# mims-harvard/ProCyon

Measured on AMD Instinct MI355X. Metric: phenotype-gen tokens/sec (ProCyon-Full greedy generation, end to end), higher is better.
Workload: dtype bf16; 1 GPU; configs[1]: ProCyon-Full (ESM2-650M + Llama-3-8B geometry=full) bf16 batch=1, 1024-residue protein, 512-token prompt, 256-token greedy generation; parallelism=single GPU

## Files before the change

procyon_amd/csrc/pcy_elem.hip:

```cpp
#include "pcy_internal.h"
#include "pcy_pick.h"

namespace {

constexpr int NT = 256;

__global__ __launch_bounds__(NT) void rmsnorm_kernel(const bf16_t* __restrict__ x, const bf16_t* __restrict__ w,
                                                     bf16_t* __restrict__ y, int d, float eps, int cast) {
  __shared__ float red[NT / 64];
  const bf16_t* xr = x + (size_t)blockIdx.x * d;
  bf16_t* yr = y + (size_t)blockIdx.x * d;
  float ss = 0.f;
  for (int k = threadIdx.x * 8; k < d; k += NT * 8) {
    const uint4 v = *reinterpret_cast<const uint4*>(xr + k);
    const uint32_t u[4] = {v.x, v.y, v.z, v.w};
#pragma unroll
    for (int j = 0; j < 4; ++j) { float a = lo_bf(u[j]), b = hi_bf(u[j]); ss += a * a + b * b; }
  }
  ss = block_sum<NT>(ss, red);
  const float rstd = rsqrtf(ss / (float)d + eps);
  for (int k = threadIdx.x * 8; k < d; k += NT * 8) {
    const uint4 v = *reinterpret_cast<const uint4*>(xr + k);
    const uint4 g = *reinterpret_cast<const uint4*>(w + k);
    const uint32_t u[4] = {v.x, v.y, v.z, v.w}, gg[4] = {g.x, g.y, g.z, g.w};
// ... 323 lines not shown
  }
  __syncthreads();
  if (tp == 0 && live) {
#pragma unroll
    for (int e = 0; e < 8; ++e) {
      float a = acc[e];
      int n = cnt[e];
#pragma unroll
      for (int q = 0; q < 3; ++q) {
        if (mode == 2) a = fmaxf(a, part[q][fg][e]);
        else { a += part[q][fg][e]; n += pcnt[q][fg][e]; }
      }
      wsum[((size_t)p * POOL_CH + ch) * d + c + e] = a;
      wcnt[((size_t)p * POOL_CH + ch) * d + c + e] = n;
    }
  }
}
__global__ __launch_bounds__(NT) void pool_finish_kernel(const float* __restrict__ wsum, const int* __restrict__ wcnt, int d, int mode,
                                                         bf16_t* __restrict__ out) {
  const int p = blockIdx.x, c = blockIdx.y * NT + threadIdx.x;
  if (c >= d) return;
  float a = wsum[(size_t)p * POOL_CH * d + c];
  int n = wcnt[(size_t)p * POOL_CH * d + c];
  for (int ch = 1; ch < POOL_CH; ++ch) {
    const float v = wsum[((size_t)p * POOL_CH + ch) * d + c];
    if (mode == 2) a = fmaxf(a, v);
    else { a += v; n += wcnt[((size_t)p * POOL_CH + ch) * d + c]; }
  }
  out[(size_t)p * d + c] = (mode == 2) ? f2bf(a) : f2bf(rbf(a) / (float)n);
}


__global__ __launch_bounds__(PICK_NT) void pick_stage1_kernel(const bf16_t* __restrict__ logits, int V, PickPartial* __restrict__ part) {
  __shared__ float redv[PICK_NT / 64];
  __shared__ int redi[PICK_NT / 64];
  __shared__ float red[PICK_NT / 64];
  const int b = blockIdx.y, c = blockIdx.x;
  const int chunk = (V + PICK_NB - 1) / PICK_NB;
  const int lo = c * chunk, hi = (lo + chunk) < V ? (lo + chunk) : V;
  const bf16_t* lg = logits + (size_t)b * V;
  float best = -INFINITY;
  int bi = 0x7fffffff;
  for (int i = lo + threadIdx.x; i < hi; i += PICK_NT) {
    const float v = bf2f(lg[i]);
    if (v > best || (v == best && i < bi)) { best = v; bi = i; }
  }
#pragma unroll
  for (int o = 32; o > 0; o >>= 1) {
    const float ov = __shfl_xor(best, o, 64);
    const int oi = __shfl_xor(bi, o, 64);
    if (ov > best || (ov == best && oi < bi)) { best = ov; bi = oi; }
  }
  const int w = threadIdx.x >> 6;
  if ((threadIdx.x & 63) == 0) { redv[w] = best; redi[w] = bi; }
  __syncthreads();
  best = redv[0]; bi = redi[0];
  for (int i = 1; i < PICK_NT / 64; ++i)
    if (redv[i] > best || (redv[i] == best && redi[i] < bi)) { best = redv[i]; bi = redi[i]; }
  float se = 0.f;
  for (int i = lo + threadIdx.x; i < hi; i += PICK_NT) se += expf(bf2f(lg[i]) - best);
  se = block_sum<PICK_NT>(se, red);
  if (threadIdx.x == 0) part[b * PICK_NB + c] = PickPartial{best, bi, best > -INFINITY ? se : 0.f, 0};
}

__global__ __launch_bounds__(256) void pick_stage2_kernel(const bf16_t* __restrict__ logits, int V, const PickPartial* __restrict__ part,
                                                          int32_t* __restrict__ next_tok, int32_t* __restrict__ tokens_out, int max_steps,
                                                          float* __restrict__ logprob, int32_t* __restrict__ step_dev, int32_t* __restrict__ pos_dev,
                                                          int advance_pos, int B, PcyStop stop) {
  __shared__ int s_unfinished;
  const int l = threadIdx.x & 63;
  if (stop.finished) {
    if (*stop.done) return;
    if (threadIdx.x == 0) s_unfinished = 0;
    __syncthreads();
  }
  const int step = *step_dev;
  for (int b = threadIdx.x >> 6; b < B; b += 4) {
    if (stop.finished && stop.finished[b]) {
      if (l == 0) { next_tok[b] = stop.eos_id; tokens_out[(size_t)b * max_steps + step] = stop.eos_id; }
      continue;
    }
    float best, se;
    int bi;
    pick_merge_row(part[b * PICK_NB + l], best, bi, se);
    if (l == 0) {
      const float lsm = pick_logprob(logits + (size_t)b * V, bi, best, se);
      logprob[b] += lsm;
      next_tok[b] = bi;
      tokens_out[(size_t)b * max_steps + step] = bi;
      if (stop.finished) {
        if (bi == stop.eos_id) stop.finished[b] = 1;
        else atomicAdd(&s_unfinished, 1);
      }
    }
  }
  __syncthreads();
  if (threadIdx.x == 0) {
    if (advance_pos) *pos_dev += 1;
    *step_dev = step + 1;
    if (stop.finished && s_unfinished == 0) {
      if (stop.n_steps_run) *stop.n_steps_run = step + 1;
      *stop.done = 1;
    }
  }
}

constexpr int SMP_NT = 1024;

__global__ __launch_bounds__(PICK_NT) void sample_stage1_kernel(const bf16_t* __restrict__ logits, int V, float temperature,
                                                                float4* __restrict__ part) {
  __shared__ float red[PICK_NT / 64];
  const int b = blockIdx.y, c = blockIdx.x;
  const int chunk = (V + PICK_NB - 1) / PICK_NB;
  const int lo = c * chunk, hi = (lo + chunk) < V ? (lo + chunk) : V;
  const bf16_t* lg = logits + (size_t)b * V;
  const bool scaled = temperature != 1.0f;
  float mr = -INFINITY, ms = -INFINITY;
  for (int i = lo + threadIdx.x; i < hi; i += PICK_NT) {
    const float v = bf2f(lg[i]);
    mr = fmaxf(mr, v);
    ms = fmaxf(ms, scaled ? rbf(v / temperature) : v);
  }
  mr = block_max<PICK_NT>(mr, red);
  ms = block_max<PICK_NT>(ms, red);
  float sr = 0.f, ss = 0.f;
  for (int i = lo + threadIdx.x; i < hi; i += PICK_NT) {
    const float v = bf2f(lg[i]);
    sr += expf(v - mr);
    ss += expf((scaled ? rbf(v / temperature) : v) - ms);
  }
  sr = block_sum<PICK_NT>(sr, red);
  ss = block_sum<PICK_NT>(ss, red);
  if (threadIdx.x == 0) part[b * PICK_NB + c] = make_float4(mr, mr > -INFINITY ? sr : 0.f, ms, ms > -INFINITY ? ss : 0.f);
}

// ... 858 lines not shown
    int acc = 0;
    for (int q = 0; q < nseq; ++q) { out[q] = acc; acc += (cu[q + 1] - cu[q] + pad - 1) / pad * pad; }
    out[nseq] = acc;
  }
}
void pcy_launch_vt_offsets(hipStream_t s, const int32_t* cu, int nseq, int pad, int32_t* vt_cu_out) {
  hipLaunchKernelGGL(vt_offsets_kernel, dim3(1), dim3(64), 0, s, cu, nseq, pad, vt_cu_out);
}
void pcy_launch_transpose_v(hipStream_t s, const bf16_t* buf, int ld, int vcol0, int nh, int dh, const int32_t* cu,
                            const int32_t* vt_cu, int nseq, int max_len, bf16_t* vt, int vt_total) {
  if (nseq <= 0) return;
  const int maxpad = (max_len + 63) / 64 * 64;
  hipLaunchKernelGGL(transpose_v_kernel, dim3((maxpad + 63) / 64, nh * dh / 64, nseq), dim3(NT), 0, s, buf, ld, vcol0, dh, cu, vt_cu, vt, vt_total);
}
size_t pcy_pool_ws_bytes(int nprot, int d) { return (size_t)nprot * POOL_CH * d * 8; }
void pcy_launch_pool(hipStream_t s, const bf16_t* h, int d, const int32_t* seg, const int32_t* rng, int nprot, int mode, bf16_t* out,
                     void* ws) {
  if (nprot <= 0) return;
  float* wsum = reinterpret_cast<float*>(ws);
  int* wcnt = reinterpret_cast<int*>(wsum + (size_t)nprot * POOL_CH * d);
  hipLaunchKernelGGL(pool_partial_kernel, dim3(nprot, (d + 511) / 512, POOL_CH), dim3(NT), 0, s, h, d, seg, rng, mode, wsum, wcnt);
  hipLaunchKernelGGL(pool_finish_kernel, dim3(nprot, (d + NT - 1) / NT), dim3(NT), 0, s, wsum, wcnt, d, mode, out);
}
void pcy_launch_pick_stage1(hipStream_t s, const bf16_t* logits, int rows, int V, void* partials) {
  if (rows > 0) hipLaunchKernelGGL(pick_stage1_kernel, dim3(PICK_NB, rows), dim3(PICK_NT), 0, s, logits, V, reinterpret_cast<PickPartial*>(partials));
}
void pcy_launch_greedy_pick(hipStream_t s, const bf16_t* logits, int B, int V, int32_t* next_tok, int32_t* tokens_out,
                            int max_steps, float* logprob, int32_t* pos_dev, int32_t* step_dev, int advance_pos, void* partials,
                            const PcyStop& stop) {
  hipLaunchKernelGGL(pick_stage1_kernel, dim3(PICK_NB, B), dim3(PICK_NT), 0, s, logits, V, reinterpret_cast<PickPartial*>(partials));
  hipLaunchKernelGGL(pick_stage2_kernel, dim3(1), dim3(256), 0, s, logits, V, reinterpret_cast<const PickPartial*>(partials), next_tok,
                     tokens_out, max_steps, logprob, step_dev, pos_dev, advance_pos, B, stop);
}
int pcy_sample_max_vocab() { return SMP_NT * SMP_KMAX; }
void pcy_launch_sample_step(hipStream_t s, const bf16_t* logits, int B, int V, float temperature, float nucleus_p, const float* uniforms,
                            unsigned* hist, bf16_t* probs_out, int32_t* next_tok, int32_t* tokens_out, int max_steps, float* logprob,
                            int32_t* pos_dev, int32_t* step_dev, int advance_pos, void* partials, bf16_t* pbits, const PcyStop& stop) {
  hipLaunchKernelGGL(sample_stage1_kernel, dim3(PICK_NB, B), dim3(PICK_NT), 0, s, logits, V, temperature, reinterpret_cast<float4*>(partials));
  hipLaunchKernelGGL(sample_probs_kernel, dim3(PICK_NB, B), dim3(PICK_NT), 0, s, logits, V, reinterpret_cast<const float4*>(partials), temperature,
                     nucleus_p > 0.f ? 1 : 0, hist, pbits, stop, probs_out ? 1 : 0);
  hipLaunchKernelGGL(sample_stage2_kernel, dim3(B), dim3(SMP_NT), 0, s, logits, V, reinterpret_cast<const float4*>(partials), temperature,
                     nucleus_p, uniforms, hist, probs_out, next_tok, tokens_out, max_steps, logprob, step_dev, B, pbits, stop);
  hipLaunchKernelGGL(sample_advance_kernel, dim3(1), dim3(64), 0, s, pos_dev, step_dev, advance_pos, stop, B);
}
void pcy_launch_copy_rows(hipStream_t s, const bf16_t* src, int lds_, bf16_t* dst, int ldd, const int32_t* rows, int nrows, int d) {
  if (nrows > 0) hipLaunchKernelGGL(copy_rows_kernel, dim3(nrows), dim3(NT), 0, s, src, lds_, dst, ldd, rows, d);
}
void pcy_launch_l2norm_rows(hipStream_t s, const bf16_t* x, bf16_t* y, int rows, int d, float eps) {
  if (rows > 0) hipLaunchKernelGGL(l2norm_rows_kernel, dim3(rows), dim3(NT), 0, s, x, y, d, eps);
}
void pcy_launch_retrieval_rank(hipStream_t s, const bf16_t* sims, int Q, int N, int k, int32_t* idx_out, bf16_t* score_out) {
  if (Q > 0 && N > 0 && k > 0)
    hipLaunchKernelGGL(retrieval_rank_kernel, dim3((N + NT - 1) / NT, Q), dim3(NT), 0, s, sims, N, k, idx_out, score_out);
}
void pcy_launch_retrieval_dot_f32(hipStream_t s, const float* query, int Q, const void* targets, int targets_bf16, int N, int D, float eps, float* sims) {
  if (Q <= 0 || N <= 0) return;
  const size_t smem = (size_t)RET_QT * D * sizeof(float);
  const dim3 grid((unsigned)((N + NT / 64 - 1) / (NT / 64) < 2048 ? (N + NT / 64 - 1) / (NT / 64) : 2048), (Q + RET_QT - 1) / RET_QT);
  if (targets_bf16) {
    static bool conf = false;
    if (!conf && smem > 65536) { (void)hipFuncSetAttribute(reinterpret_cast<const void*>(&retrieval_dot_f32_kernel<true>), hipFuncAttributeMaxDynamicSharedMemorySize, 160 * 1024 - 1024); conf = true; }
    hipLaunchKernelGGL(retrieval_dot_f32_kernel<true>, grid, dim3(NT), smem, s, query, Q, targets, N, D, eps, sims);
  } else {
    static bool conf = false;
    if (!conf && smem > 65536) { (void)hipFuncSetAttribute(reinterpret_cast<const void*>(&retrieval_dot_f32_kernel<false>), hipFuncAttributeMaxDynamicSharedMemorySize, 160 * 1024 - 1024); conf = true; }
    hipLaunchKernelGGL(retrieval_dot_f32_kernel<false>, grid, dim3(NT), smem, s, query, Q, targets, N, D, eps, sims);
// ... 28 lines not shown
```

procyon_amd/csrc/pcy_engine.hip:

```cpp
#include <stdio.h>
#include <stdlib.h>
#include <stdarg.h>
#include <string.h>
#include <dlfcn.h>
#include <vector>

#include "../../include/pcy.h"
#include "pcy_internal.h"

namespace {

thread_local char g_err[512] = "";

int fail(int code, const char* fmt, ...) {
  va_list ap;
  va_start(ap, fmt);
  vsnprintf(g_err, sizeof(g_err), fmt, ap);
  va_end(ap);
  return code;
}

#define HIP_TRY(expr)                                                                       \
  do {                                                                                      \
    hipError_t e_ = (expr);                                                                 \
// ... 156 lines not shown

int check_head_dim(const char* what, int dh, bool dh32) {
  return dh == 64 || dh == 128 || (dh32 && dh == 32) ? 0 : fail(1, "%s: head_dim %d unsupported (%s64/128)", what, dh, dh32 ? "32/" : "");
}
int check_heads(const char* what, int H, int Hkv, int dh, bool dh32) {
  if (int r = check_head_dim(what, dh, dh32)) return r;
  return Hkv < 1 || H % Hkv || !(H / Hkv == 1 || H / Hkv == 2 || H / Hkv == 4 || H / Hkv == 8) ? fail(1, "%s: H/Hkv must be 1, 2, 4 or 8", what) : 0;
}
int check_widths(const char* what, const pcy_llama_desc* m, int multiple, bool qkv_row) {
  const int HD = m->n_heads * m->head_dim, last = (qkv_row ? m->n_heads + 2 * m->n_kv_heads : m->n_kv_heads) * m->head_dim;
  if (m->d % multiple == 0 && m->ffn % multiple == 0 && HD % multiple == 0 && last % multiple == 0) return 0;
  return fail(1, "%s: d, ffn, H*dh, %s must be multiples of %d", what, qkv_row ? "(H+2Hkv)*dh" : "Hkv*dh", multiple);
}

void linear(hipStream_t s, const bf16_t* A, int lda, const bf16_t* W, const bf16_t* bias, const bf16_t* resid, int ldr,
            bf16_t* C, int ldc, int M, int N, int K, int epi, float* splitk_ws = nullptr, size_t splitk_ws_bytes = 0,
            const bf16_t* next_w = nullptr, bf16_t* next_xn = nullptr, int* fused = nullptr, float rms_eps = 0.f, int rms_cast = 0, int splitk_fill = 0) {
  if (M <= 8 && epi != EPI_SWIGLU && (resid == nullptr || ldr == ldc)) {
    PcyGemvArgs g{};
    g.W = W; g.x = A; g.y = C; g.bias = bias; g.resid = resid; g.rms_w = nullptr;
    g.N = N; g.K = K; g.B = M; g.ldx = lda; g.ldy = ldc; g.epi = epi;
    pcy_launch_gemv(s, g);
    return;
  }
  PcyGemmArgs a{};
  a.A = A; a.W = W; a.C = C; a.bias = bias; a.resid = resid;
  a.M = M; a.N = N; a.K = K; a.lda = lda; a.ldc = ldc; a.ldr = ldr; a.epi = epi;
  a.splitk_ws = splitk_ws; a.splitk_ws_bytes = splitk_ws_bytes;
  a.next_rms_w = next_w; a.next_xn = next_xn; a.fused_next = fused; a.rms_eps = rms_eps; a.rms_cast = rms_cast; a.splitk_fill = splitk_fill;
  pcy_launch_gemm(s, a);
}

unsigned long long* g_mc_trace = nullptr;
constexpr int AO_MAX_LAYERS = 128, AO_FLAGS = 64;
bool decode_nb_covers(const pcy_ctx* c, const pcy_llama_desc* m, int B, const PcySwitches& sw) {
  return B >= 2 && B <= sw.nb_max && m->d == 4096 && m->ffn == 14336 && m->n_heads == 32 && m->n_kv_heads == 8 && m->head_dim == 128 &&
         c->n_cu >= 256 && m->n_layers <= AO_MAX_LAYERS / 2;
}
bool decode_mb_covers(const pcy_ctx* c, const pcy_llama_desc* m, int B, const PcySwitches& sw) {
  return B >= 9 && B <= 32 && B <= sw.mb_max && m->d == 4096 && m->ffn == 14336 && m->n_heads == 32 && m->n_kv_heads == 8 && m->head_dim == 128 && c->n_cu >= 256;
}
size_t tag_words_per_layer(const pcy_llama_desc* m) {
  return (size_t)m->ffn + (size_t)m->d + (size_t)(m->n_heads + 2 * m->n_kv_heads) * m->head_dim + (size_t)m->n_heads * m->head_dim;
}

int ensure_sync_words(pcy_ctx* c) {
  if (!c->n_cu) {
    hipDeviceProp_t prop;
    HIP_TRY(hipGetDeviceProperties(&prop, c->device));
    c->n_cu = prop.multiProcessorCount;
  }
  if (!c->xwg_err) {
    HIP_TRY(hipHostMalloc(reinterpret_cast<void**>(&c->xwg_err), 64, hipHostMallocMapped | hipHostMallocCoherent));
    memset(c->xwg_err, 0, 64);
  }
  if (!c->ao_sync) {
    const size_t bytes = (size_t)(64 + 2 * AO_MAX_LAYERS * AO_FLAGS) * sizeof(unsigned);
    HIP_TRY(hipMalloc(reinterpret_cast<void**>(&c->ao_sync), bytes));
    HIP_TRY(hipMemset(c->ao_sync, 0, bytes));
  }
  return 0;
}
uint64_t fnv1a(uint64_t h, std::initializer_list<const void*> ptrs) {
  for (const void* p : ptrs) h = (h ^ (uint64_t)(uintptr_t)p) * 1099511628211ull;
  return h;
}
constexpr uint64_t FNV_BASIS = 1469598103934665603ull;
// ... 355 lines not shown
    launch_proj(cx, p, backend, qkv, nullptr, p.defer_qkv_finish ? &qkv_splits : nullptr);
    bool o_done = false;
    if (attn == ATTN_DECODE) {
      PcyDecAttnArgs t = attn_args(cx, p, l);
      if (qkv_splits > 1) { t.qkv_partials = cx.sk_ws; t.qkv_splits = qkv_splits; }
      o_done = p.attn_o && pcy_launch_attn_o(c->stream, t, proj_args(cx, p, o, xn_ready), c->n_cu, c->ao_sync, c->ao_sync + 64 + l * AO_FLAGS, AO_FLAGS, c->xwg_err,
                                                     c->ao_sync + 64 + (AO_MAX_LAYERS + l) * AO_FLAGS);
      if (!o_done) { t.xmin = 0; pcy_launch_attn_decode(c->stream, t); }
    } else {
      launch_attn(c->stream, attn, AttnCall{cx.qkv, cx.qkvw, cx.kv, l, cx.ao, m->n_heads * m->head_dim, cx.st->pos, (const bf16_t*)m->rope_cos, (const bf16_t*)m->rope_sin, cx.st->keep,
                                            cx.B, m->n_heads, m->n_kv_heads, m->head_dim, attn_ws});
    }
    if (!o_done) launch_proj(cx, p, backend, o, xn_ready);
    norm_if_needed(cx, feeds_xn, gu.ln, xn_ready);
    launch_proj(cx, p, backend, gu, nullptr);
    launch_proj(cx, p, backend, down, xn_ready);
  }
}
void enqueue_lm_head(const DecodeCx& cx, const DecodePlan& p, void* logits_out, int xn_ready, bool force_stream = false) {
  const pcy_llama_desc* m = cx.m;
  PcyGemvArgs h{};
  h.W = (const bf16_t*)m->lm_head; h.x = cx.x; h.y = (bf16_t*)logits_out; h.rms_w = (const bf16_t*)m->final_norm; h.rms_eps = m->rms_eps;
  h.rms_cast = m->rms_cast; h.N = m->vocab; h.K = m->d; h.B = cx.B; h.ldx = m->d; h.ldy = m->vocab; h.epi = EPI_STORE;
  if (p.batched_head && !(p.nb_on && cx.B <= 4)) {
    norm_if_needed(cx, true, m->final_norm, &xn_ready);
    h.x = cx.xn; h.rms_w = nullptr;
  } else {
    h.force_stream = p.nb_on || force_stream;
  }
  pcy_launch_gemv(cx.c->stream, h);
}

void enqueue_decode(pcy_ctx* c, const pcy_llama_desc* m, const pcy_kv_cache* kv, const pcy_gen_state* st, int B, const PcySwitches& sw, bool layers_only = false,
                    bool split = false) {
  hipStream_t s = c->stream;
  const int d = m->d, dh = m->head_dim;
  const DecodeCx cx = decode_cx(c, m, kv, st, B);
  DecodePlan p = plan_decode(c, m, kv, B, sw);
  if (split) { p.defer_qkv_finish = false; p.attn_o = false; }
  if (layers_only) {
    if (p.epoch_word) pcy_launch_bump(s, p.epoch_word);
    if (p.tag_word) pcy_launch_bump(s, p.tag_word);
  } else {
    pcy_launch_embed_tokens_dev(s, (const bf16_t*)m->embed, st->next_tok, cx.x, B, d, p.epoch_word, p.tag_word);
  }
  const size_t tag_stride = tag_words_per_layer(m);
  bool step_done = false;
  const bool try_layer = p.path == DEC_STEP_GQA || p.path == DEC_STEP_MHA || p.path == DEC_LAYERS;
  int xn_ready = 0;
  if (p.path == DEC_STEP_NB) {
    const PcyDecodeStepArgs sa = step_args(cx, c->nb_tags[B], pcy_decode_nb_tag_words(B), 2 * AO_FLAGS, pcy_decode_nb_line_words(B));
    step_done = pcy_launch_decode_step_nb(s, c->device, attn_args(cx, p, -1), block_args(cx, p.tag_word, mc_trace(sw)), mlp_args(cx, p.tag_word), sa, c->n_cu,
                                          c->ao_sync, B, sw.nb_ub);
    if (step_done) ++g_pcy_dispatch[PCY_DISPATCH_DEC_STEP_NB];
  } else if (p.path == DEC_STEP_GQA || p.path == DEC_STEP_MHA) {
    const PcyDecodeStepArgs sa = step_args(cx, c->mc_tags, tag_stride, AO_FLAGS, 32 * 256);
    step_done = pcy_launch_decode_step(s, attn_args(cx, p, -1), block_args(cx, p.tag_word, mc_trace(sw)), mlp_args(cx, p.tag_word), sa, c->n_cu,
                                       c->ao_sync);
  } else if (p.path == DEC_STEP_MB) {
    PcyMbArgs ma{};
    ma.layers = c->dev_layers; ma.n_layers = m->n_layers; ma.final_norm = (const bf16_t*)m->final_norm;
    ma.x = cx.x; ma.xn = cx.xn; ma.ao = cx.ao; ma.act = cx.act;
    ma.qkv_ws = cx.sk_ws; ma.sk_ws = cx.sk_ws + (size_t)2 * B * cx.qkvw;
    ma.kcache = (bf16_t*)kv->k; ma.vcache = (bf16_t*)kv->v; ma.kv_layer_stride = cx.layer_stride; ma.Bcache = kv->B;
    ma.pos_dev = st->pos; ma.cos_t = (const bf16_t*)m->rope_cos; ma.sin_t = (const bf16_t*)m->rope_sin; ma.keep = st->keep; ma.ld_keep = kv->Tmax;
    ma.B = B; ma.Tmax = kv->Tmax; ma.scale = 1.0f / sqrtf((float)dh); ma.rms_eps = m->rms_eps; ma.rms_cast = m->rms_cast;
    ma.flags = c->mb_flags; ma.epoch = c->mb_sync; ma.err = c->xwg_err; ma.abl = sw.mb_abl; ma.trace = mc_trace(sw);
    pcy_launch_rmsnorm(s, cx.x, (const bf16_t*)m->layers[0].ln1, cx.xn, B, d, m->rms_eps, m->rms_cast);
    if (pcy_launch_decode_step_mb(s, c->device, ma, c->n_cu)) { step_done = true; xn_ready = 1; ++g_pcy_dispatch[PCY_DISPATCH_DEC_STEP_MB]; }
  }
  int l = step_done ? m->n_layers : 0;
  for (; try_layer && l < m->n_layers; ++l) {
    const pcy_llama_layer& L = m->layers[l];
    uint32_t* tags = c->mc_tags + (size_t)l * tag_stride;
    if (!pcy_launch_decode_layer(s, attn_args(cx, p, l), block_args(cx, p.tag_word, mc_trace(sw, l), &L, tags), mlp_args(cx, p.tag_word, &L, tags), c->n_cu,
                                 c->ao_sync, c->ao_sync + 64 + (AO_MAX_LAYERS + l) * AO_FLAGS))
// ... 16 lines not shown
  const size_t step = (size_t)(*step_dev);
  const int chunks = (V + 7) / 8;
  const bool vec = (ld % 8 == 0) && ((reinterpret_cast<uintptr_t>(all) & 15) == 0);
  for (size_t i = (size_t)blockIdx.x * blockDim.x + threadIdx.x; i < (size_t)B * chunks; i += (size_t)gridDim.x * blockDim.x) {
    const int b = (int)(i / chunks), c = (int)(i % chunks);
    const bf16_t* src = logits + (size_t)b * V + c * 8;
    bf16_t* dst = all + (step * B + b) * ld + c * 8;
    if (vec && c * 8 + 8 <= V) {
      const uint32_t w0 = src[0] | ((uint32_t)src[1] << 16), w1 = src[2] | ((uint32_t)src[3] << 16);
      const uint32_t w2 = src[4] | ((uint32_t)src[5] << 16), w3 = src[6] | ((uint32_t)src[7] << 16);
      *reinterpret_cast<uint4*>(dst) = make_uint4(w0, w1, w2, w3);
    } else {
      for (int e = 0; e < 8 && c * 8 + e < V; ++e) dst[e] = src[e];
    }
  }
}
void enqueue_store_logits(hipStream_t s, const void* logits, void* all, int ld, const int32_t* step_dev, int B, int V, const int32_t* done = nullptr) {
  if (all) hipLaunchKernelGGL(store_logits_kernel, dim3(B >= 8 ? 256 : 64), dim3(256), 0, s, (const bf16_t*)logits, (bf16_t*)all, step_dev, B, V, ld > 0 ? ld : V, done);
}
PcyStop stop_of(const pcy_gen_state* st) {
  return st->finished ? PcyStop{st->finished, st->done, st->n_steps_run, st->eos_id} : PcyStop{};
}
int check_stop(const pcy_gen_state* st, int vocab, const char* what) {
  if (!st || !st->finished) return 0;
  if (!st->done) return fail(1, "%s: an EOS stop (finished != NULL) needs the done word", what);
  if (st->eos_id < 0 || st->eos_id >= vocab) return fail(1, "%s: eos_id %d outside [0, vocab %d)", what, st->eos_id, vocab);
  return 0;
}
void enqueue_pick(pcy_ctx* c, const pcy_llama_desc* m, const pcy_gen_state* st, int B, int advance_pos, int Tmax) {
  const PcyStop stop = stop_of(st);
  enqueue_store_logits(c->stream, st->logits, st->logits_all, st->logits_all_ld, st->step, B, m->vocab, stop.done);
  pcy_launch_greedy_pick(c->stream, (const bf16_t*)st->logits, B, m->vocab, st->next_tok, st->tokens_out, st->max_steps,
                         st->logprob, st->pos, st->step, advance_pos, carve_decode_ws(c->ws, m, B, Tmax).partials, stop);
}

void enqueue_sample(pcy_ctx* c, const pcy_llama_desc* m, const pcy_gen_state* st, int B, int advance_pos, int Tmax, float temperature,
                    float nucleus_p, const float* uniforms, bf16_t* probs_out) {
  hipStream_t s = c->stream;
  if (nucleus_p > 0.f) temperature = 1.0f;
  const PcyStop stop = stop_of(st);
  enqueue_store_logits(s, st->logits, st->logits_all, st->logits_all_ld, st->step, B, m->vocab, stop.done);
  void* partials = carve_decode_ws(c->ws, m, B, Tmax).partials;
  pcy_launch_sample_step(s, (const bf16_t*)st->logits, B, m->vocab, temperature, nucleus_p, uniforms, c->smp_hist, probs_out, st->next_tok,
                         st->tokens_out, st->max_steps, st->logprob, st->pos, st->step, advance_pos, partials, c->smp_pbits, stop);
}
int ensure_sample_state(pcy_ctx* c, int B, int V) {
  if ((size_t)B * V > c->smp_pbits_elems) {
    if (c->smp_pbits) { HIP_TRY(hipStreamSynchronize(c->stream)); HIP_TRY(hipFree(c->smp_pbits)); c->smp_pbits = nullptr; c->smp_pbits_elems = 0; }
    HIP_TRY(hipMalloc(reinterpret_cast<void**>(&c->smp_pbits), (size_t)B * V * 2));
    c->smp_pbits_elems = (size_t)B * V;
  }
  if (B <= c->smp_hist_rows) return 0;
  if (c->smp_hist) { HIP_TRY(hipStreamSynchronize(c->stream)); HIP_TRY(hipFree(c->smp_hist)); c->smp_hist = nullptr; }
  HIP_TRY(hipMalloc(reinterpret_cast<void**>(&c->smp_hist), (size_t)B * 65536 * sizeof(unsigned)));
  HIP_TRY(hipMemset(c->smp_hist, 0, (size_t)B * 65536 * sizeof(unsigned)));
  c->smp_hist_rows = B;
  return 0;
}

template <int MAXB>
__global__ __launch_bounds__(128) void kv_permute_kernel(bf16_t* __restrict__ kbase, bf16_t* __restrict__ vbase, const int32_t* __restrict__ rows, int B,
                                                         int Bcache, int Hkv, int Tmax, int t, int dh, const int32_t* __restrict__ t_dev, int t0, int t_off) {
  __shared__ uint4 stage[MAXB * 128];
  const int h = blockIdx.x, lw = blockIdx.y, l = lw >> 1;
  unsigned need = 0;
  bool moves = false;
// ... 1093 lines not shown
int pcy_look_draft(pcy_ctx* c, const pcy_llama_desc* m, const pcy_look_state* ls, const pcy_gen_state* st, void* embeds_out) {
  PCY_STICKY(c);
  PcyLookArgs a;
  if (int r = look_args("pcy_look_draft", ls, st, &a)) return r;
  if (!embeds_out) return fail(1, "pcy_look_draft: embeds_out is NULL");
  if (m->d % 8) return fail(1, "pcy_look_draft: d %% 8 != 0");
  pcy_launch_look_draft(c->stream, a, (const bf16_t*)m->embed, m->vocab, m->d, (bf16_t*)embeds_out);
  ++g_pcy_look[0];
  return check_launch("pcy_look_draft");
}
int pcy_look_verify(pcy_ctx* c, const pcy_llama_desc* m, const pcy_look_state* ls, const pcy_gen_state* st, const void* logits) {
  PCY_STICKY(c);
  PcyLookArgs a;
  if (int r = look_args("pcy_look_verify", ls, st, &a)) return r;
  if (!logits) return fail(1, "pcy_look_verify: logits is NULL");
  if (int r = check_stop(st, m->vocab, "pcy_look_verify")) return r;
  if (int r = c->reserve(pcy_look_verify_ws_bytes(a.W))) return r;
  pcy_launch_look_verify(c->stream, a, (const bf16_t*)logits, m->vocab, (bf16_t*)st->logits_all, st->logits_all_ld, c->ws, stop_of(st));
  ++g_pcy_look[1];
  return check_launch("pcy_look_verify");
}
unsigned long long pcy_debug_look_count(int which) { return (which == 0 || which == 1) ? g_pcy_look[which] : 0; }


int pcy_llama_greedy(pcy_ctx* c, const pcy_llama_desc* m, const pcy_kv_cache* kv, const pcy_gen_state* st, int B, int n_steps,
                     int use_graph) {
  PCY_STICKY(c);
  PcySwitches sw;
  if (m) if (int r = check_stop(st, m->vocab, "pcy_llama_greedy")) return r;
  if (int r = decode_prologue(c, m, kv, st, B, "pcy_llama_greedy", step_ws_bytes, &sw)) return r;
  DecodeGraphKey key;
  decode_graph_key(key, c, m, kv, st, B, KIND_GREEDY, sw);
  key_record(key, st);
  return run_steps(c, n_steps, use_graph != 0, "pcy_llama_greedy", key, [&] {
    enqueue_decode(c, m, kv, st, B, sw);
    enqueue_pick(c, m, st, B, 1, kv_cap(kv));
  });
}

int pcy_llama_decode_graph(pcy_ctx* c, const pcy_llama_desc* m, const pcy_kv_cache* kv, const pcy_gen_state* st, int B) {
  PCY_STICKY(c);
  PcySwitches sw;
  if (int r = decode_prologue(c, m, kv, st, B, "pcy_llama_decode_graph", step_ws_bytes, &sw)) return r;
  DecodeGraphKey key;
  decode_graph_key(key, c, m, kv, st, B, KIND_DECODE, sw);
  key_record(key, st);
  return run_steps(c, 1, true, "pcy_llama_decode_graph", key, [&] { enqueue_decode(c, m, kv, st, B, sw); });
}


static void enqueue_decode_gemm(pcy_ctx* c, const pcy_llama_desc* m, const pcy_kv_cache* kv, const pcy_gen_state* st, int B, bool mq, bool split = false) {
  const DecodeCx cx = decode_cx(c, m, kv, st, B);
  char* attn_ws = c->ws + (split ? split_ws_offset(m, kv, B) : align_up(decode_ws_bytes(m, B, kv_cap(kv)), 256));
  const DecodePlan p{};
  pcy_launch_embed_tokens_dev(c->stream, (const bf16_t*)m->embed, st->next_tok, cx.x, B, m->d);
  int xn_ready = 0;
  enqueue_layers(cx, p, BACKEND_GEMM, split ? ATTN_SPLIT : mq ? ATTN_MQ : ATTN_DECODE, attn_ws, 0, &xn_ready);
  norm_if_needed(cx, true, m->final_norm, &xn_ready);
  linear(c->stream, cx.xn, m->d, (const bf16_t*)m->lm_head, nullptr, nullptr, 0, (bf16_t*)st->logits, m->vocab, B, m->vocab, m->d, EPI_STORE);
  ++g_pcy_decode_gemm;
  if (mq) ++g_pcy_attn_mq;
  if (split) ++g_pcy_attn_split;
}

static int decode_gemm_entry(pcy_ctx* c, const pcy_llama_desc* m, const pcy_kv_cache* kv, const pcy_gen_state* st, int B, bool mq, bool split = false) {
  PCY_STICKY(c);
  const char* what = split ? "pcy_llama_decode_gemm_split" : mq ? "pcy_llama_decode_gemm_mq" : "pcy_llama_decode_gemm";
  if (int r = check_step_args(m, kv, st, B, what)) return r;
  const int H = m->n_heads, Hkv = m->n_kv_heads, dh = m->head_dim;
  if (m->layers_fp8) return fail(1, "%s: fp8 projections are not supported on this step", what);
// ... 523 lines not shown
```

procyon_amd/csrc/pcy_internal.h:

```cpp
#pragma once
#include "pcy_common.h"
#include "pcy_switch.h"

struct PcyGemvArgs {
  const bf16_t* W;
  const bf16_t* x;
  bf16_t* y;
  const bf16_t* bias;
  const bf16_t* resid;
  const bf16_t* rms_w;
  float rms_eps;
  int rms_cast;
  int N, K, B, ldx, ldy, epi;
  int plain_loads;
  float* splitk_ws; size_t splitk_ws_bytes;
  const bf16_t* next_rms_w; bf16_t* next_xn; int* fused_next;
  int* defer_finish;
  int force_stream;
  int force_mfma;
  int krot;
};
void pcy_launch_gemv(hipStream_t s, const PcyGemvArgs& a);

struct PcyGemvW8Args {
// ... 310 lines not shown
bool pcy_decode_nb_launchable(int device, int B, int Tmax, int n_cu, int ub);
int pcy_gemv_rms_threads(int N);

struct PcyMbArgs {
  const PcyLayerWeightsDev* layers; int n_layers;
  const bf16_t* final_norm;
  bf16_t* x;
  bf16_t* xn;
  bf16_t* ao;
  bf16_t* act;
  float* qkv_ws;
  float* sk_ws;
  bf16_t* kcache; bf16_t* vcache; size_t kv_layer_stride; int Bcache;
  const int32_t* pos_dev; const bf16_t* cos_t; const bf16_t* sin_t; const uint8_t* keep; int ld_keep;
  int B, Tmax; float scale, rms_eps; int rms_cast;
  unsigned* flags;
  const unsigned* epoch;
  unsigned* err;
  unsigned long long* trace;
  int abl;
};
size_t pcy_decode_mb_flag_words();
int pcy_decode_mb_ds(int B);
bool pcy_decode_mb_fits(int B, int Tmax);
bool pcy_launch_decode_step_mb(hipStream_t s, int device, const PcyMbArgs& a, int n_cu);

size_t pcy_pool_ws_bytes(int nprot, int d);
void pcy_launch_pool(hipStream_t s, const bf16_t* h, int d, const int32_t* seg, const int32_t* rng, int nprot,
                     int mode, bf16_t* out, void* ws);
void pcy_launch_greedy_pick(hipStream_t s, const bf16_t* logits, int B, int V, int32_t* next_tok, int32_t* tokens_out,
                            int max_steps, float* logprob, int32_t* pos_dev, int32_t* step_dev, int advance_pos,
                            void* partials , const PcyStop& stop = PcyStop{});
void pcy_launch_pick_stage1(hipStream_t s, const bf16_t* logits, int rows, int V, void* partials);
struct PcyLookArgs {
  int32_t* hist; int32_t* n_hist; int32_t* window; const int32_t* forced; int32_t* counters; int32_t* last;
  int cap, W, gmax, gmin;
  int32_t* pos; int32_t* step; int32_t* next_tok; int32_t* tokens_out; float* logprob; int max_steps;
};
size_t pcy_look_verify_ws_bytes(int W);
void pcy_launch_look_draft(hipStream_t s, const PcyLookArgs& a, const bf16_t* embed, int V, int d, bf16_t* embeds_out );
void pcy_launch_look_verify(hipStream_t s, const PcyLookArgs& a, const bf16_t* logits , int V, bf16_t* logits_all, int logits_all_ld,
                            void* partials , const PcyStop& stop = PcyStop{});
void pcy_launch_retrieval_dot_f32(hipStream_t s, const float* query, int Q, const void* targets, int targets_bf16, int N, int D, float eps, float* sims);
size_t pcy_retrieval_dot_smem(int D);
void pcy_launch_retrieval_rank_f32(hipStream_t s, const float* sims, int Q, int N, int k, int32_t* idx_out, float* score_out);
int pcy_sample_max_vocab();
void pcy_launch_sample_step(hipStream_t s, const bf16_t* logits, int B, int V, float temperature, float nucleus_p, const float* uniforms,
                            unsigned* hist, bf16_t* probs_out, int32_t* next_tok, int32_t* tokens_out, int max_steps, float* logprob,
                            int32_t* pos_dev, int32_t* step_dev, int advance_pos, void* partials ,
                            bf16_t* pbits , const PcyStop& stop = PcyStop{});
struct PcyBeamState {
  int32_t* out; int32_t max_len;
  float* cur; float* cur_new;
  int32_t* next_tok;
  int32_t* src;
  int32_t* anc;
  uint8_t* has_eos;
  int32_t* blk_eos; int32_t* ticket;
  int32_t* pos; int32_t* step; int32_t* done;
  int32_t eos_id;
};
size_t pcy_beam_ws_bytes(int B, int beam);
void pcy_launch_beam_step(hipStream_t s, const bf16_t* logits, int V, int B, int beam, int g, float penalty, const PcyBeamState& st,
                          void* ws);
void pcy_launch_f32_beam_step(hipStream_t s, const float* logits, int V, int B, int beam, int g, float penalty, const PcyBeamState& st,
                              void* ws);
// ... 7 lines not shown
```

procyon_amd/csrc/pcy_pick.h:

```cpp
#pragma once
#include "pcy_common.h"

constexpr int PICK_NT = 256;
constexpr int PICK_NB = 64;
struct PickPartial { float mx; int idx; float se; int pad; };

__device__ __forceinline__ void pick_merge_row(const PickPartial pp, float& best, int& bi, float& se) {
  best = pp.mx;
  bi = pp.idx;
#pragma unroll
  for (int o = 32; o > 0; o >>= 1) {
    const float ov = __shfl_xor(best, o, 64);
    const int oi = __shfl_xor(bi, o, 64);
    if (ov > best || (ov == best && oi < bi)) { best = ov; bi = oi; }
  }
  se = pp.se * expf(pp.mx - best);
  se = wave_sum(se);
}
__device__ __forceinline__ float pick_logprob(const bf16_t* __restrict__ row_logits, int bi, float best, float se) {
  return rbf((bf2f(row_logits[bi]) - best) - logf(se));
}
```

procyon_amd/csrc/pcy_switch.h:

```cpp
#pragma once
#include <stdint.h>
#include <stdlib.h>
#include <string.h>
#include <type_traits>

#define PCY_SWITCH_NAMES(X)                                                                                                                \
  X(attn_o) X(mlp_chain) X(decode_layer) X(decode_step) X(attn_qkv_finish) X(finish_norm) X(fp8_fused_norm) X(prefill_post_qkv) X(gemv_lds) \
  X(gemv_mfma4) X(fa_vrow) X(gelu_fast) X(esm_graph) X(lds_prefetch) X(decode_nb) X(decode_nb_step) X(beam_graph) X(kv_permute)             \
  X(decode_mb_step) X(beam_prefill_once) X(beam_kv_suffix) X(beam_kv_shared)
enum PcySwitch {
#define X(n) PCY_SW_##n,
  PCY_SWITCH_NAMES(X)
#undef X
  PCY_SW_COUNT
};
static_assert(PCY_SW_COUNT <= 32, "PcySwitches::off_mask holds one bit per name");

inline bool pcy_list_has(const char* list, const char* name) {
  if (!list) return false;
  const size_t n = strlen(name);
  for (const char* p = list; (p = strstr(p, name)) != nullptr; p += n)
    if ((p == list || p[-1] == ',') && (p[n] == 0 || p[n] == ',')) return true;
  return false;
}
inline bool pcy_off(const char* name) { return pcy_list_has(getenv("PCY_DISABLE"), name); }

struct PcySwitches {
  uint32_t off_mask;
  int32_t nb_max, mb_max;
  int32_t xmin[3];
  int32_t nb_ub;
  int32_t mb_abl;
  int32_t mc_trace;
  bool off(PcySwitch s) const { return (off_mask >> s) & 1u; }
  int ao_xmin(int rows) const { return xmin[rows <= 1 ? 0 : rows == 2 ? 1 : 2]; }
  bool operator==(const PcySwitches& o) const { return memcmp(this, &o, sizeof(*this)) == 0; }
  bool operator!=(const PcySwitches& o) const { return !(*this == o); }
};

static_assert(std::has_unique_object_representations<PcySwitches>::value, "no padding: equal values <=> equal bytes");

inline PcySwitches pcy_read_switches() {
// ... 21 lines not shown
```

Before: 397.4 tokens/s.

## Fuse greedy pick, logits store and next-token embedding into one tail kernel

Adds a greedy_tail kernel that computes per-chunk argmax/sum-exp partials, uses an atomic ticket so the last block merges the partials and commits the token, then writes the next step's embedding row and bumps the epoch/tag words. It also copies the logits into the all-logits buffer. This replaces the separate store-logits, pick stage1/stage2 and embed launches for each decode step. The embedding for the first step is issued once before the step loop. It relies on a grid-wide last-block ticket with release/acquire fences, which adds ordering complexity for a few fewer launches per token.

```diff
diff --git a/procyon_amd/csrc/pcy_elem.hip b/procyon_amd/csrc/pcy_elem.hip
--- a/procyon_amd/csrc/pcy_elem.hip
+++ b/procyon_amd/csrc/pcy_elem.hip
@@ -379,75 +379,75 @@
 
 
 __global__ __launch_bounds__(PICK_NT) void pick_stage1_kernel(const bf16_t* __restrict__ logits, int V, PickPartial* __restrict__ part) {
-  __shared__ float redv[PICK_NT / 64];
-  __shared__ int redi[PICK_NT / 64];
-  __shared__ float red[PICK_NT / 64];
   const int b = blockIdx.y, c = blockIdx.x;
-  const int chunk = (V + PICK_NB - 1) / PICK_NB;
-  const int lo = c * chunk, hi = (lo + chunk) < V ? (lo + chunk) : V;
-  const bf16_t* lg = logits + (size_t)b * V;
-  float best = -INFINITY;
-  int bi = 0x7fffffff;
-  for (int i = lo + threadIdx.x; i < hi; i += PICK_NT) {
-    const float v = bf2f(lg[i]);
-    if (v > best || (v == best && i < bi)) { best = v; bi = i; }
-  }
-#pragma unroll
-  for (int o = 32; o > 0; o >>= 1) {
-    const float ov = __shfl_xor(best, o, 64);
-    const int oi = __shfl_xor(bi, o, 64);
-    if (ov > best || (ov == best && oi < bi)) { best = ov; bi = oi; }
-  }
-  const int w = threadIdx.x >> 6;
-  if ((threadIdx.x & 63) == 0) { redv[w] = best; redi[w] = bi; }
-  __syncthreads();
-  best = redv[0]; bi = redi[0];
-  for (int i = 1; i < PICK_NT / 64; ++i)
-    if (redv[i] > best || (redv[i] == best && redi[i] < bi)) { best = redv[i]; bi = redi[i]; }
-  float se = 0.f;
-  for (int i = lo + threadIdx.x; i < hi; i += PICK_NT) se += expf(bf2f(lg[i]) - best);
-  se = block_sum<PICK_NT>(se, red);
-  if (threadIdx.x == 0) part[b * PICK_NB + c] = PickPartial{best, bi, best > -INFINITY ? se : 0.f, 0};
+  const PickPartial pp = pick_chunk_partial(logits + (size_t)b * V, V, c);
+  if (threadIdx.x == 0) part[b * PICK_NB + c] = pp;
 }
 
 __global__ __launch_bounds__(256) void pick_stage2_kernel(const bf16_t* __restrict__ logits, int V, const PickPartial* __restrict__ part,
                                                           int32_t* __restrict__ next_tok, int32_t* __restrict__ tokens_out, int max_steps,
                                                           float* __restrict__ logprob, int32_t* __restrict__ step_dev, int32_t* __restrict__ pos_dev,
                                                           int advance_pos, int B, PcyStop stop) {
-  __shared__ int s_unfinished;
-  const int l = threadIdx.x & 63;
-  if (stop.finished) {
-    if (*stop.done) return;
-    if (threadIdx.x == 0) s_unfinished = 0;
-    __syncthreads();
-  }
-  const int step = *step_dev;
-  for (int b = threadIdx.x >> 6; b < B; b += 4) {
-    if (stop.finished && stop.finished[b]) {
-      if (l == 0) { next_tok[b] = stop.eos_id; tokens_out[(size_t)b * max_steps + step] = stop.eos_id; }
-      continue;
-    }
-    float best, se;
-    int bi;
-    pick_merge_row(part[b * PICK_NB + l], best, bi, se);
-    if (l == 0) {
-      const float lsm = pick_logprob(logits + (size_t)b * V, bi, best, se);
-      logprob[b] += lsm;
-      next_tok[b] = bi;
-      tokens_out[(size_t)b * max_steps + step] = bi;
-      if (stop.finished) {
-        if (bi == stop.eos_id) stop.finished[b] = 1;
-        else atomicAdd(&s_unfinished, 1);
-      }
-    }
-  }
-  __syncthreads();
-  if (threadIdx.x == 0) {
-    if (advance_pos) *pos_dev += 1;
-    *step_dev = step + 1;
-    if (stop.finished && s_unfinished == 0) {
-      if (stop.n_steps_run) *stop.n_steps_run = step + 1;
-      *stop.done = 1;
+  pick_commit_rows<false>(logits, V, part, next_tok, tokens_out, max_steps, logprob, step_dev, pos_dev, advance_pos, B, stop);
+}
+
+__global__ __launch_bounds__(PICK_NT) void greedy_tail_kernel(PcyTailArgs a) {
+  __shared__ unsigned s_ticket;
+  const int b = blockIdx.y, c = blockIdx.x, tid = threadIdx.x;
+  const bool live = !(a.stop.finished && *a.stop.done);
+  const size_t step = (size_t)(*a.step_dev);
+  const bf16_t* lg = a.logits + (size_t)b * a.V;
+  PickPartial pp{};
+  if (live) pp = pick_chunk_partial(lg, a.V, c);
+  if (tid == 0) {
+    if (live) {
+      unsigned long long* dst = reinterpret_cast<unsigned long long*>(reinterpret_cast<PickPartial*>(a.partials) + b * PICK_NB + c);
+      __hip_atomic_store(dst, (unsigned long long)__float_as_uint(pp.mx) | ((unsigned long long)(uint32_t)pp.idx << 32), __ATOMIC_RELAXED, __HIP_MEMORY_SCOPE_AGENT);
+      __hip_atomic_store(dst + 1, (unsigned long long)__float_as_uint(pp.se), __ATOMIC_RELAXED, __HIP_MEMORY_SCOPE_AGENT);
+    }
+    __builtin_amdgcn_fence(__ATOMIC_RELEASE, "agent");
+    asm volatile("s_waitcnt vmcnt(0)" ::: "memory");
+    s_ticket = atomicInc(a.ticket, gridDim.x * gridDim.y - 1);
+  }
+  __syncthreads();
+  const bool last = s_ticket == gridDim.x * gridDim.y - 1;
+  if (last) {
+    if (tid == 0) {
+      __builtin_amdgcn_fence(__ATOMIC_ACQUIRE, "agent");
+      asm volatile("s_waitcnt vmcnt(0)" ::: "memory");
+    }
+    __syncthreads();
+    if (live)
+      pick_commit_rows<true>(a.logits, a.V, reinterpret_cast<const PickPartial*>(a.partials), a.next_tok, a.tokens_out, a.max_steps, a.logprob, a.step_dev, a.pos_dev, a.advance_pos, a.B, a.stop);
+    __syncthreads();
+    for (int r = 0; r < a.B; ++r) {
+      const bf16_t* src = a.embed + (size_t)a.next_tok[r] * a.d;
+      for (int k = tid * 8; k < a.d; k += PICK_NT * 8) *reinterpret_cast<uint4*>(a.x + (size_t)r * a.d + k) = *reinterpret_cast<const uint4*>(src + k);
+    }
+    if (tid == 0) {
+      if (a.epoch) *a.epoch += 1;
+      if (a.tag) *a.tag += 1;
+    }
+  }
+  if (!live || !a.all) return;
+  const int groups = (a.V + 7) / 8;
+  const bool vec = (a.ld % 8 == 0) && ((reinterpret_cast<uintptr_t>(a.all) & 15) == 0);
+  const bool vec_src = (reinterpret_cast<uintptr_t>(lg) & 15) == 0;
+  bf16_t* row = a.all + (step * a.B + b) * a.ld;
+  for (int g = c * PICK_NT + tid; g < groups; g += PICK_NB * PICK_NT) {
+    const bf16_t* src = lg + g * 8;
+    bf16_t* dst = row + g * 8;
+    if (vec && g * 8 + 8 <= a.V) {
+      uint4 v;
+      if (vec_src) {
+        v = *reinterpret_cast<const uint4*>(src);
+      } else {
+        v = make_uint4(src[0] | ((uint32_t)src[1] << 16), src[2] | ((uint32_t)src[3] << 16), src[4] | ((uint32_t)src[5] << 16),
+                       src[6] | ((uint32_t)src[7] << 16));
+      }
+      *reinterpret_cast<uint4*>(dst) = v;
+    } else {
+      for (int e = 0; e < 8 && g * 8 + e < a.V; ++e) dst[e] = src[e];
     }
   }
 }
@@ -1372,6 +1372,9 @@
   hipLaunchKernelGGL(pick_stage2_kernel, dim3(1), dim3(256), 0, s, logits, V, reinterpret_cast<const PickPartial*>(partials), next_tok,
                      tokens_out, max_steps, logprob, step_dev, pos_dev, advance_pos, B, stop);
 }
+void pcy_launch_greedy_tail(hipStream_t s, const PcyTailArgs& a) {
+  hipLaunchKernelGGL(greedy_tail_kernel, dim3(PICK_NB, a.B), dim3(PICK_NT), 0, s, a);
+}
 int pcy_sample_max_vocab() { return SMP_NT * SMP_KMAX; }
 void pcy_launch_sample_step(hipStream_t s, const bf16_t* logits, int B, int V, float temperature, float nucleus_p, const float* uniforms,
                             unsigned* hist, bf16_t* probs_out, int32_t* next_tok, int32_t* tokens_out, int max_steps, float* logprob,
diff --git a/procyon_amd/csrc/pcy_engine.hip b/procyon_amd/csrc/pcy_engine.hip
--- a/procyon_amd/csrc/pcy_engine.hip
+++ b/procyon_amd/csrc/pcy_engine.hip
@@ -212,7 +212,7 @@
 }
 
 unsigned long long* g_mc_trace = nullptr;
-constexpr int AO_MAX_LAYERS = 128, AO_FLAGS = 64;
+constexpr int AO_MAX_LAYERS = 128, AO_FLAGS = 64, AO_TICKET = 32;
 bool decode_nb_covers(const pcy_ctx* c, const pcy_llama_desc* m, int B, const PcySwitches& sw) {
   return B >= 2 && B <= sw.nb_max && m->d == 4096 && m->ffn == 14336 && m->n_heads == 32 && m->n_kv_heads == 8 && m->head_dim == 128 &&
          c->n_cu >= 256 && m->n_layers <= AO_MAX_LAYERS / 2;
@@ -634,7 +634,7 @@
 }
 
 void enqueue_decode(pcy_ctx* c, const pcy_llama_desc* m, const pcy_kv_cache* kv, const pcy_gen_state* st, int B, const PcySwitches& sw, bool layers_only = false,
-                    bool split = false) {
+                    bool split = false, bool x_ready = false) {
   hipStream_t s = c->stream;
   const int d = m->d, dh = m->head_dim;
   const DecodeCx cx = decode_cx(c, m, kv, st, B);
@@ -643,7 +643,7 @@
   if (layers_only) {
     if (p.epoch_word) pcy_launch_bump(s, p.epoch_word);
     if (p.tag_word) pcy_launch_bump(s, p.tag_word);
-  } else {
+  } else if (!x_ready) {
     pcy_launch_embed_tokens_dev(s, (const bf16_t*)m->embed, st->next_tok, cx.x, B, d, p.epoch_word, p.tag_word);
   }
   const size_t tag_stride = tag_words_per_layer(m);
@@ -726,6 +726,24 @@
   enqueue_store_logits(c->stream, st->logits, st->logits_all, st->logits_all_ld, st->step, B, m->vocab, stop.done);
   pcy_launch_greedy_pick(c->stream, (const bf16_t*)st->logits, B, m->vocab, st->next_tok, st->tokens_out, st->max_steps,
                          st->logprob, st->pos, st->step, advance_pos, carve_decode_ws(c->ws, m, B, Tmax).partials, stop);
+}
+
+constexpr int GREEDY_TAIL_MAX_ROWS = 8;
+unsigned long long g_pcy_greedy_tail = 0;
+void enqueue_greedy_tail(pcy_ctx* c, const pcy_llama_desc* m, const pcy_kv_cache* kv, const pcy_gen_state* st, int B, const PcySwitches& sw) {
+  const DecodeWs w = carve_decode_ws(c->ws, m, B, kv_cap(kv));
+  const DecodePlan p = plan_decode(c, m, kv, B, sw);
+  PcyTailArgs a{};
+  a.logits = (const bf16_t*)st->logits; a.V = m->vocab; a.B = B;
+  a.all = (bf16_t*)st->logits_all; a.ld = st->logits_all_ld > 0 ? st->logits_all_ld : m->vocab;
+  a.partials = w.partials;
+  a.next_tok = st->next_tok; a.tokens_out = st->tokens_out; a.max_steps = st->max_steps; a.logprob = st->logprob;
+  a.step_dev = st->step; a.pos_dev = st->pos; a.advance_pos = 1;
+  a.embed = (const bf16_t*)m->embed; a.x = w.x; a.d = m->d;
+  a.epoch = p.epoch_word; a.tag = p.tag_word; a.ticket = c->ao_sync + AO_TICKET;
+  a.stop = stop_of(st);
+  pcy_launch_greedy_tail(c->stream, a);
+  ++g_pcy_greedy_tail;
 }
 
 void enqueue_sample(pcy_ctx* c, const pcy_llama_desc* m, const pcy_gen_state* st, int B, int advance_pos, int Tmax, float temperature,
@@ -1885,10 +1903,24 @@
   DecodeGraphKey key;
   decode_graph_key(key, c, m, kv, st, B, KIND_GREEDY, sw);
   key_record(key, st);
+  const bool tail = !sw.off(PCY_SW_greedy_tail) && B <= GREEDY_TAIL_MAX_ROWS;
+  if (tail && n_steps > 0) {
+    const DecodePlan p = plan_decode(c, m, kv, B, sw);
+    pcy_launch_embed_tokens_dev(c->stream, (const bf16_t*)m->embed, st->next_tok, carve_decode_ws(c->ws, m, B, kv_cap(kv)).x, B, m->d, p.epoch_word, p.tag_word);
+  }
   return run_steps(c, n_steps, use_graph != 0, "pcy_llama_greedy", key, [&] {
-    enqueue_decode(c, m, kv, st, B, sw);
-    enqueue_pick(c, m, st, B, 1, kv_cap(kv));
+    enqueue_decode(c, m, kv, st, B, sw, false, false, tail);
+    if (tail) enqueue_greedy_tail(c, m, kv, st, B, sw);
+    else enqueue_pick(c, m, st, B, 1, kv_cap(kv));
   });
+}
+unsigned long long pcy_debug_greedy_tail(pcy_ctx* c, int which) {
+  if (which == 0) return g_pcy_greedy_tail;
+  unsigned word = 0;
+  if (which != 1 || !c || !c->ao_sync || hipStreamSynchronize(c->stream) != hipSuccess ||
+      hipMemcpy(&word, c->ao_sync + AO_TICKET, sizeof(word), hipMemcpyDeviceToHost) != hipSuccess)
+    return ~0ull;
+  return word;
 }
 
 int pcy_llama_decode_graph(pcy_ctx* c, const pcy_llama_desc* m, const pcy_kv_cache* kv, const pcy_gen_state* st, int B) {
diff --git a/procyon_amd/csrc/pcy_internal.h b/procyon_amd/csrc/pcy_internal.h
--- a/procyon_amd/csrc/pcy_internal.h
+++ b/procyon_amd/csrc/pcy_internal.h
@@ -366,6 +366,16 @@
                             int max_steps, float* logprob, int32_t* pos_dev, int32_t* step_dev, int advance_pos,
                             void* partials , const PcyStop& stop = PcyStop{});
 void pcy_launch_pick_stage1(hipStream_t s, const bf16_t* logits, int rows, int V, void* partials);
+struct PcyTailArgs {
+  const bf16_t* logits; int V, B;
+  bf16_t* all; int ld;
+  void* partials;
+  int32_t *next_tok, *tokens_out; int max_steps; float* logprob; int32_t *step_dev, *pos_dev; int advance_pos;
+  const bf16_t* embed; bf16_t* x; int d;
+  unsigned *epoch, *tag, *ticket;
+  PcyStop stop;
+};
+void pcy_launch_greedy_tail(hipStream_t s, const PcyTailArgs& a);
 struct PcyLookArgs {
   int32_t* hist; int32_t* n_hist; int32_t* window; const int32_t* forced; int32_t* counters; int32_t* last;
   int cap, W, gmax, gmin;
diff --git a/procyon_amd/csrc/pcy_pick.h b/procyon_amd/csrc/pcy_pick.h
--- a/procyon_amd/csrc/pcy_pick.h
+++ b/procyon_amd/csrc/pcy_pick.h
@@ -1,9 +1,39 @@
 #pragma once
-#include "pcy_common.h"
+#include "pcy_internal.h"
 
 constexpr int PICK_NT = 256;
 constexpr int PICK_NB = 64;
 struct PickPartial { float mx; int idx; float se; int pad; };
+
+__device__ __forceinline__ PickPartial pick_chunk_partial(const bf16_t* __restrict__ lg, int V, int c) {
+  __shared__ float redv[PICK_NT / 64];
+  __shared__ int redi[PICK_NT / 64];
+  __shared__ float red[PICK_NT / 64];
+  const int chunk = (V + PICK_NB - 1) / PICK_NB;
+  const int lo = c * chunk, hi = (lo + chunk) < V ? (lo + chunk) : V;
+  float best = -INFINITY;
+  int bi = 0x7fffffff;
+  for (int i = lo + threadIdx.x; i < hi; i += PICK_NT) {
+    const float v = bf2f(lg[i]);
+    if (v > best || (v == best && i < bi)) { best = v; bi = i; }
+  }
+#pragma unroll
+  for (int o = 32; o > 0; o >>= 1) {
+    const float ov = __shfl_xor(best, o, 64);
+    const int oi = __shfl_xor(bi, o, 64);
+    if (ov > best || (ov == best && oi < bi)) { best = ov; bi = oi; }
+  }
+  const int w = threadIdx.x >> 6;
+  if ((threadIdx.x & 63) == 0) { redv[w] = best; redi[w] = bi; }
+  __syncthreads();
+  best = redv[0]; bi = redi[0];
+  for (int i = 1; i < PICK_NT / 64; ++i)
+    if (redv[i] > best || (redv[i] == best && redi[i] < bi)) { best = redv[i]; bi = redi[i]; }
+  float se = 0.f;
+  for (int i = lo + threadIdx.x; i < hi; i += PICK_NT) se += expf(bf2f(lg[i]) - best);
+  se = block_sum<PICK_NT>(se, red);
+  return PickPartial{best, bi, best > -INFINITY ? se : 0.f, 0};
+}
 
 __device__ __forceinline__ void pick_merge_row(const PickPartial pp, float& best, int& bi, float& se) {
   best = pp.mx;
@@ -20,3 +50,52 @@
 __device__ __forceinline__ float pick_logprob(const bf16_t* __restrict__ row_logits, int bi, float best, float se) {
   return rbf((bf2f(row_logits[bi]) - best) - logf(se));
 }
+
+template <bool AGENT>
+__device__ __forceinline__ void pick_commit_rows(const bf16_t* __restrict__ logits, int V, const PickPartial* part, int32_t* __restrict__ next_tok,
+                                                 int32_t* __restrict__ tokens_out, int max_steps, float* __restrict__ logprob,
+                                                 int32_t* __restrict__ step_dev, int32_t* __restrict__ pos_dev, int advance_pos, int B, PcyStop stop) {
+  __shared__ int s_unfinished;
+  const int l = threadIdx.x & 63;
+  if (stop.finished) {
+    if (*stop.done) return;
+    if (threadIdx.x == 0) s_unfinished = 0;
+    __syncthreads();
+  }
+  const int step = *step_dev;
+  for (int b = threadIdx.x >> 6; b < B; b += 4) {
+    if (stop.finished && stop.finished[b]) {
+      if (l == 0) { next_tok[b] = stop.eos_id; tokens_out[(size_t)b * max_steps + step] = stop.eos_id; }
+      continue;
+    }
+    PickPartial pp;
+    if (AGENT) {
+      const uint4 u = ld16_agent(part + b * PICK_NB + l);
+      pp = PickPartial{__uint_as_float(u.x), (int)u.y, __uint_as_float(u.z), 0};
+    } else {
+      pp = part[b * PICK_NB + l];
+    }
+    float best, se;
+    int bi;
+    pick_merge_row(pp, best, bi, se);
+    if (l == 0) {
+      const float lsm = pick_logprob(logits + (size_t)b * V, bi, best, se);
+      logprob[b] += lsm;
+      next_tok[b] = bi;
+      tokens_out[(size_t)b * max_steps + step] = bi;
+      if (stop.finished) {
+        if (bi == stop.eos_id) stop.finished[b] = 1;
+        else atomicAdd(&s_unfinished, 1);
+      }
+    }
+  }
+  __syncthreads();
+  if (threadIdx.x == 0) {
+    if (advance_pos) *pos_dev += 1;
+    *step_dev = step + 1;
+    if (stop.finished && s_unfinished == 0) {
+      if (stop.n_steps_run) *stop.n_steps_run = step + 1;
+      *stop.done = 1;
+    }
+  }
+}
diff --git a/procyon_amd/csrc/pcy_switch.h b/procyon_amd/csrc/pcy_switch.h
--- a/procyon_amd/csrc/pcy_switch.h
+++ b/procyon_amd/csrc/pcy_switch.h
@@ -7,7 +7,7 @@
 #define PCY_SWITCH_NAMES(X)                                                                                                                \
   X(attn_o) X(mlp_chain) X(decode_layer) X(decode_step) X(attn_qkv_finish) X(finish_norm) X(fp8_fused_norm) X(prefill_post_qkv) X(gemv_lds) \
   X(gemv_mfma4) X(fa_vrow) X(gelu_fast) X(esm_graph) X(lds_prefetch) X(decode_nb) X(decode_nb_step) X(beam_graph) X(kv_permute)             \
-  X(decode_mb_step) X(beam_prefill_once) X(beam_kv_suffix) X(beam_kv_shared)
+  X(decode_mb_step) X(beam_prefill_once) X(beam_kv_suffix) X(beam_kv_shared) X(greedy_tail)
 enum PcySwitch {
 #define X(n) PCY_SW_##n,
   PCY_SWITCH_NAMES(X)
```

Measured after the change: 399.1 tokens/s (median of 6 runs). No clear change (+0.4%).
